# ECP-ExaGraph/miniVite

Hardware: NVIDIA B200
Metric: louvain_phase_edges_per_sec (higher is better)
Workload: dtype f64

## Files before the change

__graft_entry__.py:

```python
import os
import subprocess
import sys

ROOT = os.path.dirname(os.path.abspath(__file__))
PKG = os.path.join(ROOT, "minivite_b200")
CSRC = os.path.join(PKG, "csrc")
LIBDIR = os.path.join(PKG, "lib")
BINDIR = os.path.join(ROOT, "bin")
if ROOT not in sys.path:
    sys.path.insert(0, ROOT)

NVCC_FLAGS = ["-gencode", "arch=compute_100a,code=sm_100a", "-lineinfo", "-O3", "-std=c++17", "-fmad=false",
              "-Xcompiler", "-fPIC,-ffp-contract=off,-pthread"]
HOST_FLAGS = ["-std=c++17", "-O3", "-fopenmp", "-ffp-contract=off", "-fPIC", "-Wall"]


def _newer(target, sources):
    if not os.path.exists(target):
        return True
    t = os.path.getmtime(target)
    return any(os.path.getmtime(s) > t for s in sources)


def _srcs(*rel):
    return [os.path.join(CSRC, r) for r in rel]


def build_host_only():
    os.makedirs(LIBDIR, exist_ok=True)
    host_src = _srcs("host/hostlib.cpp", "host/rgg.hpp", "host/graph.hpp", "host/binio.hpp")
    out = os.path.join(LIBDIR, "libmvhost.so")
    if _newer(out, host_src):
        subprocess.check_call(["g++"] + HOST_FLAGS + ["-shared", "-o", out, host_src[0]])
    from oracle import oracle as O
    O.build()


def build():
    import fcntl
    os.makedirs(LIBDIR, exist_ok=True)
    lk = os.open(os.path.join(LIBDIR, ".build.lock"), os.O_RDONLY | os.O_CREAT, 0o644)
    try:
        fcntl.flock(lk, fcntl.LOCK_EX)
        _build_locked()
    finally:
        os.close(lk)


def _build_locked():
    build_host_only()
    inc = os.path.join(ROOT, "include", "mvgpu.h")
    cu_src = _srcs("mvgpu.cu", "narrow.cpp", "kernels.cuh", "scan_pipe.cuh", "rgg_gpu.cuh", "nccl_dyn.h") + [inc]
    out = os.path.join(LIBDIR, "libmvgpu.so")
    if _newer(out, cu_src):
        subprocess.check_call(["nvcc"] + NVCC_FLAGS + ["-shared", "-o", out, cu_src[0], cu_src[1], "-ldl", "-lpthread"])
    main_src = _srcs("host/main.cpp", "host/louvain.hpp", "host/rgg.hpp", "host/graph.hpp", "host/binio.hpp") + [inc]
    if all(os.path.exists(s) for s in main_src):
        os.makedirs(BINDIR, exist_ok=True)
        exe = os.path.join(BINDIR, "miniVite_b200")
        if _newer(exe, main_src + [out]):
            subprocess.check_call(["g++"] + HOST_FLAGS + ["-I", os.path.join(ROOT, "include"), "-o", exe, main_src[0],
                                                         "-L", LIBDIR, "-lmvgpu", "-Wl,-rpath,$ORIGIN/../minivite_b200/lib"])
    if os.path.isdir("/root/reference"):
        subprocess.check_call([sys.executable, os.path.join(ROOT, "oracle", "build_ref.py"), "--gpu"])
    import minivite_b200
    from minivite_b200 import gpu, hostgraph
    hostgraph.lib()
    L = gpu.lib()
    for name in gpu.EXPORTS:
        getattr(L, name)


def smoke():
    build()
    import numpy as np
    from minivite_b200 import gpu, hostgraph
    from oracle import oracle as O
    ss = hostgraph.generate_rgg(16384, 1)
    sh = ss.shards[0]
    g = gpu.LouvainGPU(0, 0, 1)
    g.set_option("trace", 1)
    g.upload(sh.nv, sh.parts, sh.rowptr, sh.edges)
    mod, iters = g.louvain(-1.0, 1.0e-6)
    comm = g.communities()
    tr = g.trace()
# ... 14 lines not shown
```

include/mvgpu.h:

```cpp
#ifndef MVGPU_H
#define MVGPU_H

#include <stdint.h>

#ifdef __cplusplus
extern "C" {
#endif

typedef struct mvgpu_ctx mvgpu_ctx;

#define MVGPU_UNIQUE_ID_BYTES 128

typedef struct {
  double modularity;
  int64_t moved;
  uint64_t chash;
} mvgpu_iter_trace;

typedef struct {
  double total_s;
  double setup_s;
  double scan_s;
  double fold_s;
  double exchange_s;
// ... 8 lines not shown
  int64_t h2d_bytes;
} mvgpu_timings;

const char *mvgpu_last_error(void);
int mvgpu_device_count(void);

int mvgpu_create(mvgpu_ctx **ctx, int device, int rank, int nranks);
int mvgpu_destroy(mvgpu_ctx *ctx);

int mvgpu_get_unique_id(void *id128);
int mvgpu_comm_init(mvgpu_ctx *ctx, const void *id128);

int mvgpu_upload_shard(mvgpu_ctx *ctx, int64_t nv_global, const int64_t *parts, int64_t lnv, int64_t lne,
                       const int64_t *edge_indices, const void *edge_list);
int mvgpu_attach_shard_device(mvgpu_ctx *ctx, int64_t nv_global, const int64_t *parts, int64_t lnv, int64_t lne,
                              const int64_t *d_edge_indices, const void *d_edge_list);

int mvgpu_generate_rgg_shard(mvgpu_ctx *ctx, int64_t nv_global, int unit_weight, int64_t *lne_out);
int mvgpu_generate_rgg_shard_ex(mvgpu_ctx *ctx, int64_t nv_global, int unit_weight, int lcg, double random_edge_percent,
                                int64_t *lne_out);
int mvgpu_download_shard(mvgpu_ctx *ctx, int64_t *edge_indices, void *edge_list);

int mvgpu_louvain(mvgpu_ctx *ctx, double lower, double thresh, int *iters, double *modularity);

int mvgpu_get_communities(mvgpu_ctx *ctx, int64_t *out);
int mvgpu_get_communities_device(mvgpu_ctx *ctx, const int32_t **d_out);

int mvgpu_set_option(mvgpu_ctx *ctx, const char *name, int64_t value);
int mvgpu_get_trace(mvgpu_ctx *ctx, int max_entries, mvgpu_iter_trace *out, int *n);
int mvgpu_get_timings(mvgpu_ctx *ctx, mvgpu_timings *out);
int mvgpu_get_scan_times(mvgpu_ctx *ctx, int max_entries, double *out, int *n);
int mvgpu_get_constant(mvgpu_ctx *ctx, double *out);
int mvgpu_get_shard_info(mvgpu_ctx *ctx, int64_t *info6);

int mvgpu_upload_shard32(mvgpu_ctx *ctx, int32_t nv_global, const int32_t *parts, int32_t lnv, int32_t lne,
                         const int32_t *edge_indices, const void *edge_list8);
int mvgpu_louvain32(mvgpu_ctx *ctx, float lower, float thresh, int *iters, float *modularity);
int mvgpu_get_communities32(mvgpu_ctx *ctx, int32_t *out);

int mvgpu_dist_louvain_method(int device, int64_t nv, int64_t ne_local, const int64_t *edge_indices,
                              const void *edge_list, double lower, double thresh, int *iters,
                              double *modularity, int64_t *comm_out);

#ifdef __cplusplus
}
#endif
#endif
```

minivite_b200/csrc/kernels.cuh:

```cuda
#pragma once
#include <cooperative_groups.h>
#include <cuda_runtime.h>
#include <stdint.h>

namespace mv {

#ifndef MV_TILE_V
#define MV_TILE_V 128
#endif
#ifndef MV_ECAP
#define MV_ECAP 2048
#endif
constexpr int kTileV = MV_TILE_V;
constexpr int kECap = MV_ECAP;
#ifndef MV_STAGE_U
#define MV_STAGE_U 6
#endif
constexpr int kStageU = MV_STAGE_U;
constexpr int kMaxRanks = 16;

struct Edge16 { long long tail; double weight; };
struct CommW { long long size; double degree; };

struct Acc {
// ... 748 lines not shown
    } else {
      double tw = 0.0, sl = 0.0;
      for (uint32_t e = e0; e < e1; e++) {
        const double w = weights[e];
        tw += w;
        if (tails[e] == v) sl += w;
      }
      vdeg[v] = tw;
      self_d[v] = (double)(long long)sl;
      any_self |= (sl != 0.0);
      CommW c; c.size = 1; c.degree = tw;
      cinfo_w[v] = c;
      usize[v] = 0; udeg[v] = 0.0;
      tw_sum += tw;
    }
  }
  tw_sum = warp_sum(tw_sum);
  if (UNIT) sq_sum = warp_sum(sq_sum);
  any_self = __any_sync(0xffffffffu, any_self);
  if (bad) *unordered = 1;
  if ((threadIdx.x & 31) == 0) {
    if (UNIT && sq_sum) atomicAdd(&acc0->la2_u, sq_sum);
    if (tw_sum != 0.0) atomicAdd(total_weight, tw_sum);
    if (any_self) atomicOr(has_self, 1u);
  }
}

__global__ void __launch_bounds__(256) k_collect_heavy(int lnv, const uint32_t *rowptr, unsigned int heavy_deg, int32_t *list,
                                                       unsigned int *count) {
  for (int v = blockIdx.x * blockDim.x + threadIdx.x; v < lnv; v += gridDim.x * blockDim.x)
    if (rowptr[v + 1] - rowptr[v] > heavy_deg) list[atomicAdd(count, 1u)] = v;
}

#ifndef MV_BFS_SUB
#define MV_BFS_SUB 4
#endif
constexpr unsigned int kBfsRegionBits = 22;
constexpr unsigned int kBfsUnreached = 0xFFFFFFFFu;

__global__ void __launch_bounds__(256) k_msbfs(int lnv, const uint32_t *rowptr, const int32_t *tails, uint32_t *key,
                                               int region_stride, int max_levels, unsigned int *level_flags) {
  namespace cg = cooperative_groups;
  cg::grid_group grid = cg::this_grid();
  const int gtid = blockIdx.x * blockDim.x + threadIdx.x, gsz = gridDim.x * blockDim.x;
  for (int v = gtid; v < lnv; v += gsz)
    key[v] = (v % region_stride == 0) ? (unsigned int)(v / region_stride) : kBfsUnreached;
  grid.sync();
  const int lane = threadIdx.x & 31;
  constexpr int kBfsSub = MV_BFS_SUB, kBfsLanes = 32 / kBfsSub;
  __shared__ uint32_t s_front[256 / 32][32][3];
  uint32_t(*front)[3] = s_front[threadIdx.x >> 5];
  for (int level = 0; level < max_levels; level++) {
    bool any = false;
    for (int vb = (gtid - lane); vb < lnv; vb += gsz) {
      const int v = vb + lane;
      unsigned int k = kBfsUnreached;
      if (v < lnv) k = __ldcg(key + v);
      const bool active = (k != kBfsUnreached) && ((k >> kBfsRegionBits) == (unsigned int)level);
      const unsigned int m = __ballot_sync(0xffffffffu, active);
      if (m == 0) continue;
      any = true;
      if (active) {
        const int slot = __popc(m & ((1u << lane) - 1u));
        front[slot][0] = ((unsigned int)(level + 1) << kBfsRegionBits) | (k & ((1u << kBfsRegionBits) - 1));
        front[slot][1] = rowptr[v];
        front[slot][2] = rowptr[v + 1];
      }
      __syncwarp();
      const int cnt = __popc(m);
      for (int i = lane / kBfsLanes; i < cnt; i += kBfsSub) {
        const unsigned int nk = front[i][0];
        const uint32_t e1 = front[i][2];
        for (uint32_t e = front[i][1] + (lane % kBfsLanes); e < e1; e += kBfsLanes) {
          const int w = tails[e];
          if (w < lnv && __ldcg(key + w) > nk) atomicMin(&key[w], nk);
        }
      }
      __syncwarp();
    }
    if (__syncthreads_or(any) && threadIdx.x == 0) level_flags[level] = 1;
    grid.sync();
    if (__ldcg(level_flags + level) == 0) break;
  }
}

constexpr unsigned int kBfsLevelBits = 8;
__global__ void __launch_bounds__(256) k_bfs_sortkeys(int lnv, const uint32_t *key, uint32_t *sortkey, int32_t *ids,
                                                      unsigned int unreached_key) {
  for (int v = blockIdx.x * blockDim.x + threadIdx.x; v < lnv; v += gridDim.x * blockDim.x) {
    const unsigned int k = key[v];
    unsigned int sk;
    if (k == kBfsUnreached) sk = unreached_key;
    else {
      const unsigned int region = k & ((1u << kBfsRegionBits) - 1), level = min(k >> kBfsRegionBits, (1u << kBfsLevelBits) - 1u);
      sk = (region << kBfsLevelBits) | level;
    }
    sortkey[v] = sk;
    ids[v] = v;
  }
}

__global__ void __launch_bounds__(256) k_perm_inverse(int lnv, const int32_t *perm, long long base, int32_t *inv, int32_t *lab,
                                                      const uint32_t *rowptr_old, uint32_t *deg_new) {
  for (int i = blockIdx.x * blockDim.x + threadIdx.x; i <= lnv; i += gridDim.x * blockDim.x) {
    if (i == lnv) { deg_new[i] = 0; continue; }
    const int o = perm[i];
    inv[o] = i;
    lab[i] = (int32_t)(base + o);
    deg_new[i] = rowptr_old[o + 1] - rowptr_old[o];
  }
}

__global__ void __launch_bounds__(256) k_permute_adj(int lnv, const int32_t *perm, const int32_t *inv, const uint32_t *rowptr_old,
                                                     const int32_t *tails_old, const double *w_old, const uint32_t *rowptr_new,
                                                     int32_t *tails_new, double *w_new, int nlow, unsigned int *unordered) {
  const int lane = threadIdx.x & 7;
  const int tile = (blockIdx.x * blockDim.x + threadIdx.x) >> 3, ntiles = (gridDim.x * blockDim.x) >> 3;
  bool bad = false;
  for (int i = tile; i < lnv; i += ntiles) {
    const int o = perm[i];
    const uint32_t s0 = rowptr_old[o], s1 = rowptr_old[o + 1], d0 = rowptr_new[i];
    for (uint32_t k = lane; k < s1 - s0; k += 8) {
      const int t = tails_old[s0 + k];
      if (k && !tails_ascend(tails_old[s0 + k - 1], t, lnv, nlow)) bad = true;
      tails_new[d0 + k] = (t < lnv) ? inv[t] : t;
      if (w_old) w_new[d0 + k] = w_old[s0 + k];
    }
  }
  if (bad) *unordered = 1;
}

__global__ void __launch_bounds__(256) k_span_sample(int lnv, const uint32_t *rowptr, const int32_t *tails, int stride,
                                                     unsigned long long *span_sum, unsigned long long *span_cnt) {
  unsigned long long s = 0, c = 0;
  for (int v = (blockIdx.x * blockDim.x + threadIdx.x) * stride; v < lnv; v += gridDim.x * blockDim.x * stride) {
    const uint32_t e1 = rowptr[v + 1];
    for (uint32_t e = rowptr[v]; e < e1; e++) {
      const int t = tails[e];
      if (t < lnv) { s += (unsigned long long)abs(t - v); c++; }
    }
  }
  s = warp_sum(s); c = warp_sum(c);
  if ((threadIdx.x & 31) == 0 && c) { atomicAdd(span_sum, s); atomicAdd(span_cnt, c); }
}

template <bool MULTI>
__global__ void __launch_bounds__(256) k_final_labels(int lnv, const int32_t *cur, const int32_t *perm, ScanParams p, int32_t *out) {
  for (int i = blockIdx.x * blockDim.x + threadIdx.x; i < lnv; i += gridDim.x * blockDim.x) {
    const int c = cur[i];
    out[perm ? perm[i] : i] = label_of<MULTI>(p, c);
  }
}

struct P2PState {
  unsigned long long arrive[kMaxRanks];
  unsigned long long vals[2][kMaxRanks][4];
  unsigned int error;
  unsigned int pad_;
};
// ... 89 lines not shown
```

minivite_b200/csrc/mvgpu.cu:

```cuda
#include <cuda_runtime.h>
#include <unistd.h>

#include <algorithm>
#include <atomic>
#include <cmath>
#include <cstdio>
#include <cstring>
#include <cub/cub.cuh>
#include <random>
#include <string>
#include <thread>
#include <vector>

#include "../../include/mvgpu.h"
#include "host_comm.hpp"
#include "kernels.cuh"
#include "scan_pipe.cuh"
#include "scan_queue.cuh"
#include "nccl_dyn.h"
#include "rgg_gpu.cuh"

extern "C" void mv_narrow_edges(const void *edge_records, long long n, long long nv, long long base, long long bound,
                                int32_t *dst, long long *nremote, int *bad);

// ... 58 lines not shown
  int device = 0, rank = 0, nranks = 1;
  cudaStream_t stream = nullptr;
  int num_sms = 148;
  ncclComm_t comm = nullptr;
  mvhost::HostComm hc;
  long long nv_global = 0, lnv = 0, lne = 0, base = 0, bound = 0;
  std::vector<long long> parts;
  const long long *d_rowptr64 = nullptr;
  const Edge16 *d_edges = nullptr;
  DevBuf<long long> in_rowptr;
  DevBuf<Edge16> in_edges;
  DevBuf<long long> gen_rowptr;
  DevBuf<Edge16> gen_edges;
  DevBuf<int32_t> in_tails32;
  DevBuf<Edge16> raw_ring;
  long long raw_chunks = 0;
  DevBuf<long long> wide;
  void *h_bounce[2] = {nullptr, nullptr};
  const int32_t *d_tails32 = nullptr;
  long long in_nremote = 0;
  void *h_stage = nullptr;
  size_t h_stage_cap = 0;
  const uint32_t *a_rowptr = nullptr;
  const int32_t *a_tails = nullptr;
  const double *a_weights = nullptr;
  bool have_graph = false;
  DevBuf<uint32_t> rowptr;
  DevBuf<int32_t> tails;
  DevBuf<double> weights;
  DevBuf<int32_t> self_i;
  DevBuf<uint32_t> bfs_key, sortkey, sortkey2, deg_new, rowptr2;
  DevBuf<int32_t> ids, perm, inv, lab, tails2, final_orig;
  DevBuf<double> weights2;
  DevBuf<unsigned int> level_flags;
  bool reordered = false;
  int relabel = 0;
  double reorder_s = 0.0;
  DevBuf<double> self_d, vdeg;
  DevBuf<int32_t> comm_a, comm_b;
  DevBuf<uint32_t> cdeg;
  DevBuf<int32_t> csize;
  DevBuf<unsigned long long> upd;
  DevBuf<CommW> cinfo_w;
  DevBuf<long long> usize;
  DevBuf<double> udeg;
  DevBuf<Acc> acc;
  DevBuf<unsigned char> scratch;
  DevBuf<unsigned char> cub_tmp, coll_tmp;
  DevBuf<long long> sorted_tmp;
  DevBuf<long long> remote_list, ghost_gid, send_gid;
  DevBuf<uint32_t> remote_pos;
  DevBuf<int32_t> send_lid, send_buf;
  long long nghost = 0, nsend = 0;
  std::vector<long long> rcount, scount, roff, soff;
  DevBuf<int32_t> heavy_list, hkeys, hvals_i;
  DevBuf<double> hvals_d;
  DevBuf<unsigned long long> heavy_off;
  long long nheavy = 0, maxdeg = 0;
  int scan_has_self = 0, scan_heavy_deg = kECap;
  int scan_kernel = 4;
  bool simple_sorted = false;
  DevBuf<P2PState> p2p;
  P2PPeers pp;
  PushTable push[2];
  unsigned long long p2p_epoch = 0;
  bool p2p_zeroed = false;
  int32_t *peer_comm[2][kMaxRanks];
// ... 410 lines not shown
    TRY(coll_alltoallv_dev(c, c->ghost_gid.p, c->rcount, c->roff, c->send_gid.p, c->scount, c->soff, sizeof(long long)));
    if (c->nsend) {
      k_gid_to_lid<<<grid_for(c->nsend, 256, nsm), 256, 0, s>>>(c->send_gid.p, (int)c->nsend, c->base, c->send_lid.p);
      c->tm.kernel_launches++;
    }
  }

  c->reordered = false;
  c->relabel = 0;
  {
    int want = c->opt_reorder == 1 ? 1 : 0;
    if (c->opt_reorder == 2 && lnv >= 65536) {
      k_span_sample<<<grid_for(lnv / 64 + 1, 256, nsm), 256, 0, s>>>((int)lnv, src_rowptr, src_tails, 64, &d_sc->span_sum, &d_sc->span_cnt);
      c->tm.kernel_launches++;
      unsigned long long sp2[2];
      CK(cudaMemcpyAsync(sp2, &d_sc->span_sum, sizeof sp2, cudaMemcpyDeviceToHost, s));
      CK(cudaStreamSynchronize(s));
      if (sp2[1] > 0 && (double)sp2[0] / (double)sp2[1] > (double)lnv / 64.0) want = 1;
    }
    int any = want;
    if (c->nranks > 1) {
      long long hv = want;
      TRY(coll_allreduce_i64(c, &hv, 1, true));
      any = hv != 0;
    }
    c->relabel = any;
    if (any && lnv > 0) {
      cudaEvent_t r0 = get_event(c, 2), r1 = get_event(c, 3);
      CK(cudaEventRecord(r0, s));
      TRY(c->perm.ensure(lnv)); TRY(c->inv.ensure(lnv)); TRY(c->lab.ensure(lnv)); TRY(c->ids.ensure(lnv));
      TRY(c->bfs_key.ensure(lnv)); TRY(c->sortkey.ensure(lnv)); TRY(c->sortkey2.ensure(lnv));
      TRY(c->deg_new.ensure(lnv + 1)); TRY(c->rowptr2.ensure(lnv + 1 + 40)); TRY(c->tails2.ensure(lne + 4));
      if (!c->unit) TRY(c->weights2.ensure(lne + 4));
      const int max_levels = 1023;
      TRY(c->level_flags.ensure(max_levels + 1));
      CK(cudaMemsetAsync(c->level_flags.p, 0, sizeof(unsigned int) * (max_levels + 1), s));
      if (want) {
        int occ = 0;
        CK(cudaOccupancyMaxActiveBlocksPerMultiprocessor(&occ, k_msbfs, 256, 0));
        if (occ < 1) return fail("k_msbfs cannot be made resident");
        int ilnv = (int)lnv, stride = c->opt_region, ml = max_levels;
        const uint32_t *rp = src_rowptr; const int32_t *tl = src_tails; uint32_t *key = c->bfs_key.p; unsigned int *lf = c->level_flags.p;
        void *args[] = {&ilnv, &rp, &tl, &key, &stride, &ml, &lf};
        CK(cudaLaunchCooperativeKernel((void *)k_msbfs, dim3(occ * nsm), dim3(256), args, 0, s));
        const long long nregions = (lnv + stride - 1) / stride;
        int sort_bits = (int)kBfsLevelBits;
        while ((1LL << (sort_bits - (int)kBfsLevelBits)) <= nregions && sort_bits < 32) sort_bits++;
        const unsigned int unreached_key = sort_bits >= 32 ? 0xFFFFFFFFu : ((1u << sort_bits) - 1u);
        k_bfs_sortkeys<<<grid_for(lnv, 256, nsm), 256, 0, s>>>((int)lnv, c->bfs_key.p, c->sortkey.p, c->ids.p, unreached_key);
        size_t tb = 0;
        cub::DeviceRadixSort::SortPairs(nullptr, tb, c->sortkey.p, c->sortkey2.p, c->ids.p, c->perm.p, (int)lnv, 0, sort_bits, s);
        TRY(c->cub_tmp.ensure(tb));
        tb = c->cub_tmp.cap;
        CK(cub::DeviceRadixSort::SortPairs(c->cub_tmp.p, tb, c->sortkey.p, c->sortkey2.p, c->ids.p, c->perm.p, (int)lnv, 0, sort_bits, s));
        c->tm.kernel_launches += 3;
      } else {
        k_bfs_sortkeys<<<grid_for(lnv, 256, nsm), 256, 0, s>>>((int)lnv, c->bfs_key.p, c->sortkey.p, c->perm.p, 0xFFFFFFFFu);
        c->tm.kernel_launches++;
      }
      k_perm_inverse<<<grid_for(lnv + 1, 256, nsm), 256, 0, s>>>((int)lnv, c->perm.p, c->base, c->inv.p, c->lab.p, src_rowptr, c->deg_new.p);
      c->tm.kernel_launches++;
      if (want) {
        size_t tb = 0;
        cub::DeviceScan::ExclusiveSum(nullptr, tb, c->deg_new.p, c->rowptr2.p, (int)lnv + 1, s);
        TRY(c->cub_tmp.ensure(tb));
        tb = c->cub_tmp.cap;
        CK(cub::DeviceScan::ExclusiveSum(c->cub_tmp.p, tb, c->deg_new.p, c->rowptr2.p, (int)lnv + 1, s));
        k_permute_adj<<<grid_for(lnv * 8, 256, nsm, 16), 256, 0, s>>>((int)lnv, c->perm.p, c->inv.p, src_rowptr, src_tails, src_weights,
                                                                    c->rowptr2.p, c->tails2.p, c->unit ? nullptr : c->weights2.p,
                                                                    (int)c->roff[c->rank], &d_sc->unordered);
        c->tm.kernel_launches += 2;
        src_rowptr = c->rowptr2.p;
        src_tails = c->tails2.p;
        src_weights = c->unit ? nullptr : c->weights2.p;
        c->reordered = true;
      }
      CK(cudaEventRecord(r1, s));
    }
    if (c->relabel && c->nsend) {
      k_apply_inv<<<grid_for(c->nsend, 256, nsm), 256, 0, s>>>(c->send_lid.p, (int)c->nsend, c->inv.p);
      c->tm.kernel_launches++;
    }
  }

  c->a_rowptr = src_rowptr; c->a_tails = src_tails; c->a_weights = src_weights;

  const long long nslots = lnv + c->nghost;
  TRY(c->comm_a.ensure(std::max(nslots, lnv + nremote)));
  TRY(c->comm_b.ensure(std::max(nslots, lnv + nremote)));
  if (c->unit) { TRY(c->cdeg.ensure(lnv)); TRY(c->csize.ensure(lnv)); TRY(c->upd.ensure(lnv)); TRY(c->self_i.ensure(lnv)); }
  else { TRY(c->cinfo_w.ensure(lnv)); TRY(c->usize.ensure(lnv)); TRY(c->udeg.ensure(lnv)); TRY(c->vdeg.ensure(lnv)); TRY(c->self_d.ensure(lnv)); }
  TRY(c->acc.ensure((size_t)c->opt_max_iters + 2));
  CK(cudaMemsetAsync(c->acc.p, 0, sizeof(Acc) * ((size_t)c->opt_max_iters + 2), s));

  if (c->unit)
    k_vertex_init<true><<<grid_for(lnv, 256, nsm), 256, 0, s>>>((int)lnv, c->base, c->a_rowptr, c->a_tails, nullptr, c->comm_a.p,
                                                              c->cdeg.p, c->csize.p, c->upd.p, nullptr, nullptr, nullptr, nullptr,
                                                              c->self_i.p, nullptr, &d_sc->total_weight, &d_sc->has_self,
                                                              (int)c->roff[c->rank], c->reordered ? nullptr : &d_sc->unordered, c->acc.p);
  else
    k_vertex_init<false><<<grid_for(lnv, 256, nsm), 256, 0, s>>>((int)lnv, c->base, c->a_rowptr, c->a_tails, c->a_weights, c->comm_a.p,
// ... 357 lines not shown
      const std::string kv = all.substr(pos, end - pos);
      pos = end + 1;
      const size_t eq = kv.find('=');
      if (kv.empty()) continue;
      if (eq == std::string::npos || mvgpu_set_option(c, kv.substr(0, eq).c_str(), atoll(kv.c_str() + eq + 1))) {
        const std::string msg = "MVGPU_OPTIONS: bad entry '" + kv + "'" + (eq == std::string::npos ? "" : ": " + g_err);
        mvgpu_destroy(c);
        return fail(msg);
      }
    }
  }
  *out = c;
  return 0;
}

int mvgpu_destroy(mvgpu_ctx *c) {
  if (!c) return 0;
  cudaSetDevice(c->device);
  if (c->stream) cudaStreamSynchronize(c->stream);
  for (void *p : c->ipc_opened) cudaIpcCloseMemHandle(p);
  if (c->comm) g_nccl.CommDestroy(c->comm);
  c->hc.close_comm();
  for (cudaEvent_t e : c->events) cudaEventDestroy(e);
  if (c->h_stage) cudaFreeHost(c->h_stage);
  c->in_tails32.release(); c->wide.release(); c->raw_ring.release();
  for (int b = 0; b < 2; b++) if (c->h_bounce[b]) cudaFreeHost(c->h_bounce[b]);
  c->gen_rowptr.release(); c->gen_edges.release();
  c->in_rowptr.release(); c->in_edges.release(); c->rowptr.release(); c->tails.release(); c->weights.release();
  c->self_i.release(); c->self_d.release(); c->vdeg.release(); c->comm_a.release(); c->comm_b.release();
  c->cdeg.release(); c->csize.release(); c->upd.release(); c->cinfo_w.release(); c->usize.release(); c->udeg.release(); c->acc.release();
  c->scratch.release(); c->cub_tmp.release(); c->coll_tmp.release(); c->sorted_tmp.release(); c->remote_list.release(); c->remote_pos.release(); c->ghost_gid.release(); c->send_gid.release();
  c->bfs_key.release(); c->sortkey.release(); c->sortkey2.release(); c->deg_new.release(); c->rowptr2.release();
  c->ids.release(); c->perm.release(); c->inv.release(); c->lab.release(); c->tails2.release(); c->final_orig.release();
  c->weights2.release(); c->level_flags.release();
  c->p2p.release();
  c->send_lid.release(); c->send_buf.release(); c->heavy_list.release(); c->hkeys.release(); c->hvals_i.release();
  c->hvals_d.release(); c->heavy_off.release();
  if (c->h_pin) cudaFreeHost(c->h_pin);
  if (c->stream) cudaStreamDestroy(c->stream);
  delete c;
  return 0;
}

int mvgpu_get_unique_id(void *id128) {
  static_assert(sizeof(ncclUniqueId) == MVGPU_UNIQUE_ID_BYTES, "ncclUniqueId size");
  if (!mvnccl::load(g_nccl, g_err)) {
    FILE *f = fopen("/dev/urandom", "rb");
    if (!f || fread(id128, 1, MVGPU_UNIQUE_ID_BYTES, f) != MVGPU_UNIQUE_ID_BYTES) { if (f) fclose(f); return 1; }
    fclose(f);
    return 0;
  }
  ncclUniqueId id;
  NK(g_nccl.GetUniqueId(&id));
  memcpy(id128, &id, sizeof id);
  return 0;
}

int mvgpu_comm_init(mvgpu_ctx *c, const void *id128) {
  if (!c) return fail("null ctx");
  if (c->nranks == 1) return 0;
  if (c->opt_host_transport) {
    std::string err;
    if (c->hc.open(id128, c->rank, c->nranks, err)) return fail(err);
    return 0;
  }
  if (!mvnccl::load(g_nccl, g_err)) return 1;
  CK(cudaSetDevice(c->device));
// ... 360 lines not shown
  if (!c || !n) return fail("null argument");
  const int k = std::min<int>(max_entries, (int)c->trace.size());
  if (out && k > 0) memcpy(out, c->trace.data(), sizeof(mvgpu_iter_trace) * k);
  *n = (int)c->trace.size();
  return 0;
}

int mvgpu_get_scan_times(mvgpu_ctx *c, int max_entries, double *out, int *n) {
  if (!c || !n) return fail("null argument");
  const int k = std::min<int>(max_entries, (int)c->scan_times.size());
  if (out && k > 0) memcpy(out, c->scan_times.data(), sizeof(double) * k);
  *n = (int)c->scan_times.size();
  return 0;
}

int mvgpu_get_timings(mvgpu_ctx *c, mvgpu_timings *out) {
  if (!c || !out) return fail("null argument");
  *out = c->tm;
  return 0;
}

int mvgpu_get_constant(mvgpu_ctx *c, double *out) {
  if (!c || !out) return fail("null argument");
  *out = c->constant;
  return 0;
}

int mvgpu_get_shard_info(mvgpu_ctx *c, int64_t *info6) {
  if (!c || !info6) return fail("null argument");
  info6[0] = c->lnv; info6[1] = c->lne; info6[2] = c->nghost; info6[3] = c->nsend; info6[4] = c->nheavy; info6[5] = c->maxdeg;
  return 0;
}

int mvgpu_upload_shard32(mvgpu_ctx *c, int32_t nv_global, const int32_t *parts, int32_t lnv, int32_t lne,
                         const int32_t *edge_indices, const void *edge_list8) {
  if (!c || !parts || !edge_indices || (lne && !edge_list8)) return fail("null argument");
  CK(cudaSetDevice(c->device));
  std::vector<int64_t> parts64(parts, parts + c->nranks + 1);
  TRY(set_graph(c, nv_global, parts64.data(), lnv, lne));
  c->f32 = true;
  DevBuf<Edge8> e8;
  DevBuf<int32_t> rp32;
  TRY(e8.ensure((size_t)lne)); TRY(rp32.ensure((size_t)lnv + 1));
  TRY(c->in_edges.ensure(lne)); TRY(c->in_rowptr.ensure(lnv + 1));
  cudaEvent_t a = get_event(c, 0), b = get_event(c, 1);
  CK(cudaEventRecord(a, c->stream));
  CK(cudaMemcpyAsync(rp32.p, edge_indices, sizeof(int32_t) * ((size_t)lnv + 1), cudaMemcpyHostToDevice, c->stream));
  if (lne) CK(cudaMemcpyAsync(e8.p, edge_list8, sizeof(Edge8) * (size_t)lne, cudaMemcpyHostToDevice, c->stream));
  k_widen_shard32<<<grid_for(std::max<long long>(lne, lnv + 1), 256, c->num_sms, 16), 256, 0, c->stream>>>(e8.p, lne, rp32.p, lnv, c->in_edges.p,
                                                                                                      c->in_rowptr.p);
  CK(cudaEventRecord(b, c->stream));
  CK(cudaEventSynchronize(b));
  float ms = 0;
  CK(cudaEventElapsedTime(&ms, a, b));
  c->h2d_s = ms * 1e-3;
  c->h2d_bytes = (long long)sizeof(int32_t) * (lnv + 1) + (long long)sizeof(Edge8) * lne;
  c->d_rowptr64 = c->in_rowptr.p;
  c->d_edges = c->in_edges.p;
  c->d_tails32 = nullptr;
  return 0;
}

int mvgpu_louvain32(mvgpu_ctx *c, float lower, float thresh, int *iters, float *modularity) {
  if (!c || !iters || !modularity) return fail("null argument");
  if (!c->f32) return fail("mvgpu_louvain32 needs a shard uploaded with mvgpu_upload_shard32");
  double mod = 0.0;
// ... 30 lines not shown
```

minivite_b200/gpu.py:

```python
import ctypes
import os

import numpy as np

_LIB_PATH = os.environ.get("MVGPU_LIB") or os.path.join(os.path.dirname(os.path.abspath(__file__)), "lib", "libmvgpu.so")
UNIQUE_ID_BYTES = 128

TRACE_DTYPE = np.dtype([("modularity", "<f8"), ("moved", "<i8"), ("chash", "<u8")])


class Timings(ctypes.Structure):
    _fields_ = [("total_s", ctypes.c_double), ("setup_s", ctypes.c_double), ("scan_s", ctypes.c_double),
                ("fold_s", ctypes.c_double), ("exchange_s", ctypes.c_double), ("h2d_s", ctypes.c_double),
                ("scan_launches", ctypes.c_int64), ("kernel_launches", ctypes.c_int64),
                ("iters", ctypes.c_int32), ("unit_weight", ctypes.c_int32), ("reorder_s", ctypes.c_double),
                ("reordered", ctypes.c_int32), ("scan_kernel_chosen", ctypes.c_int32), ("h2d_bytes", ctypes.c_int64)]

    def as_dict(self):
        return {k: getattr(self, k) for k, _ in self._fields_}


EXPORTS = ["mvgpu_last_error", "mvgpu_device_count", "mvgpu_create", "mvgpu_destroy", "mvgpu_get_unique_id",
           "mvgpu_comm_init", "mvgpu_upload_shard", "mvgpu_attach_shard_device", "mvgpu_generate_rgg_shard", "mvgpu_generate_rgg_shard_ex",
           "mvgpu_download_shard", "mvgpu_louvain",
           "mvgpu_get_communities", "mvgpu_get_communities_device", "mvgpu_upload_shard32", "mvgpu_louvain32", "mvgpu_get_communities32", "mvgpu_set_option", "mvgpu_get_trace",
           "mvgpu_get_timings", "mvgpu_get_scan_times", "mvgpu_get_constant", "mvgpu_get_shard_info", "mvgpu_dist_louvain_method"]

_lib = None


def lib():
    global _lib
    if _lib is None:
        if not os.path.exists(_LIB_PATH):
            raise RuntimeError(f"{_LIB_PATH} missing: the CUDA extension is not built "
                               "(python -c 'import __graft_entry__ as g; g.build()'); there is no CPU fallback")
        L = ctypes.CDLL(_LIB_PATH)
        vp, i64, dbl, ci = ctypes.c_void_p, ctypes.c_int64, ctypes.c_double, ctypes.c_int
        L.mvgpu_last_error.restype = ctypes.c_char_p
        L.mvgpu_create.argtypes = [ctypes.POINTER(vp), ci, ci, ci]
        L.mvgpu_destroy.argtypes = [vp]
        L.mvgpu_get_unique_id.argtypes = [vp]
        L.mvgpu_comm_init.argtypes = [vp, vp]
        L.mvgpu_upload_shard.argtypes = [vp, i64, vp, i64, i64, vp, vp]
        L.mvgpu_attach_shard_device.argtypes = [vp, i64, vp, i64, i64, vp, vp]
        L.mvgpu_generate_rgg_shard.argtypes = [vp, i64, ci, ctypes.POINTER(i64)]
        L.mvgpu_generate_rgg_shard_ex.argtypes = [vp, i64, ci, ci, ctypes.c_double, ctypes.POINTER(i64)]
        L.mvgpu_download_shard.argtypes = [vp, vp, vp]
        L.mvgpu_louvain.argtypes = [vp, dbl, dbl, ctypes.POINTER(ci), ctypes.POINTER(dbl)]
        L.mvgpu_get_communities.argtypes = [vp, vp]
        L.mvgpu_upload_shard32.argtypes = [vp, ctypes.c_int32, vp, ctypes.c_int32, ctypes.c_int32, vp, vp]
        L.mvgpu_louvain32.argtypes = [vp, ctypes.c_float, ctypes.c_float, ctypes.POINTER(ci), ctypes.POINTER(ctypes.c_float)]
        L.mvgpu_get_communities32.argtypes = [vp, vp]
        L.mvgpu_get_communities_device.argtypes = [vp, ctypes.POINTER(vp)]
        L.mvgpu_set_option.argtypes = [vp, ctypes.c_char_p, i64]
        L.mvgpu_get_trace.argtypes = [vp, ci, vp, ctypes.POINTER(ci)]
        L.mvgpu_get_timings.argtypes = [vp, ctypes.POINTER(Timings)]
        L.mvgpu_get_scan_times.argtypes = [vp, ci, vp, ctypes.POINTER(ci)]
        L.mvgpu_get_constant.argtypes = [vp, ctypes.POINTER(dbl)]
        L.mvgpu_get_shard_info.argtypes = [vp, vp]
        L.mvgpu_dist_louvain_method.argtypes = [ci, i64, i64, vp, vp, dbl, dbl, ctypes.POINTER(ci),
                                                ctypes.POINTER(dbl), vp]
        _lib = L
    return _lib


class MvgpuError(RuntimeError):
    pass


def _ck(rc):
    if rc != 0:
        raise MvgpuError(lib().mvgpu_last_error().decode(errors="replace"))


def device_count():
    n = lib().mvgpu_device_count()
    if n < 0:
        raise MvgpuError(lib().mvgpu_last_error().decode(errors="replace"))
    return n


def get_unique_id():
    buf = ctypes.create_string_buffer(UNIQUE_ID_BYTES)
    _ck(lib().mvgpu_get_unique_id(buf))
    return buf.raw


class LouvainGPU:

    def __init__(self, device=0, rank=0, nranks=1):
        self._h = ctypes.c_void_p()
        self.rank, self.nranks, self.device = rank, nranks, device
# ... 76 lines not shown
        _ck(lib().mvgpu_get_communities(self._h, out.ctypes.data))
        return out[:self.lnv]

    def trace(self):
        n = ctypes.c_int(0)
        _ck(lib().mvgpu_get_trace(self._h, 0, None, ctypes.byref(n)))
        out = np.zeros(n.value, dtype=TRACE_DTYPE)
        if n.value:
            _ck(lib().mvgpu_get_trace(self._h, n.value, out.ctypes.data, ctypes.byref(n)))
        return out

    def timings(self):
        t = Timings()
        _ck(lib().mvgpu_get_timings(self._h, ctypes.byref(t)))
        return t.as_dict()

    def scan_times(self):
        n = ctypes.c_int(0)
        _ck(lib().mvgpu_get_scan_times(self._h, 0, None, ctypes.byref(n)))
        out = np.zeros(n.value, dtype=np.float64)
        if n.value:
            _ck(lib().mvgpu_get_scan_times(self._h, n.value, out.ctypes.data, ctypes.byref(n)))
        return out

    def constant(self):
        v = ctypes.c_double(0)
        _ck(lib().mvgpu_get_constant(self._h, ctypes.byref(v)))
        return v.value

    def shard_info(self):
        info = (ctypes.c_int64 * 6)()
        _ck(lib().mvgpu_get_shard_info(self._h, info))
        return dict(zip(["lnv", "lne", "nghost", "nsend", "nheavy", "maxdeg"], [int(x) for x in info]))

    def close(self):
        if self._h:
            lib().mvgpu_destroy(self._h)
            self._h = ctypes.c_void_p()

    def __del__(self):
        try:
            self.close()
        except Exception:
            pass


def dist_louvain_method(me, nprocs, shard, lower=-1.0, thresh=1.0e-6, device=None, unique_id=None, want_comm=False):
    g = LouvainGPU(device if device is not None else me, me, nprocs)
    try:
        if nprocs > 1:
            g.comm_init(unique_id)
        g.upload(shard.nv, shard.parts, shard.rowptr, shard.edges)
        mod, iters = g.louvain(lower, thresh)
        if want_comm:
            return mod, iters, g.communities()
        return mod, iters
    finally:
        g.close()
```

Measured before the change: 191.9 billion.

## Replace level-scan multi-source BFS with frontier-queue BFS and warp-balanced adjacency permute

The reordering BFS used to rescan every vertex at every level to find the active frontier. It now keeps explicit frontier queues, with warp-level load-balanced edge expansion and claims staged in shared memory. Once the frontier becomes small, the remaining levels finish in a single CTA, so small levels avoid grid-wide syncs. The adjacency permutation kernel is rewritten so each warp handles 32 rows with load-balanced edge distribution instead of eight lanes per row. A permutation-export API is also added. Claiming vertices via atomicMin can change which region wins compared with the previous relaxation, and that could alter the ordering.

```diff
diff --git a/__graft_entry__.py b/__graft_entry__.py
--- a/__graft_entry__.py
+++ b/__graft_entry__.py
@@ -50,7 +50,8 @@
 def _build_locked():
     build_host_only()
     inc = os.path.join(ROOT, "include", "mvgpu.h")
-    cu_src = _srcs("mvgpu.cu", "narrow.cpp", "kernels.cuh", "scan_pipe.cuh", "rgg_gpu.cuh", "nccl_dyn.h") + [inc]
+    cu_src = _srcs("mvgpu.cu", "narrow.cpp", "kernels.cuh", "scan_pipe.cuh", "scan_queue.cuh", "rgg_gpu.cuh", "nccl_dyn.h",
+                    "host_comm.hpp") + [inc]
     out = os.path.join(LIBDIR, "libmvgpu.so")
     if _newer(out, cu_src):
         subprocess.check_call(["nvcc"] + NVCC_FLAGS + ["-shared", "-o", out, cu_src[0], cu_src[1], "-ldl", "-lpthread"])
diff --git a/include/mvgpu.h b/include/mvgpu.h
--- a/include/mvgpu.h
+++ b/include/mvgpu.h
@@ -64,6 +64,7 @@
 int mvgpu_get_scan_times(mvgpu_ctx *ctx, int max_entries, double *out, int *n);
 int mvgpu_get_constant(mvgpu_ctx *ctx, double *out);
 int mvgpu_get_shard_info(mvgpu_ctx *ctx, int64_t *info6);
+int mvgpu_get_permutation(mvgpu_ctx *ctx, int32_t *perm_out);
 
 int mvgpu_upload_shard32(mvgpu_ctx *ctx, int32_t nv_global, const int32_t *parts, int32_t lnv, int32_t lne,
                          const int32_t *edge_indices, const void *edge_list8);
diff --git a/minivite_b200/csrc/kernels.cuh b/minivite_b200/csrc/kernels.cuh
--- a/minivite_b200/csrc/kernels.cuh
+++ b/minivite_b200/csrc/kernels.cuh
@@ -804,55 +804,117 @@
     if (rowptr[v + 1] - rowptr[v] > heavy_deg) list[atomicAdd(count, 1u)] = v;
 }
 
-#ifndef MV_BFS_SUB
-#define MV_BFS_SUB 4
-#endif
 constexpr unsigned int kBfsRegionBits = 22;
 constexpr unsigned int kBfsUnreached = 0xFFFFFFFFu;
-
-__global__ void __launch_bounds__(256) k_msbfs(int lnv, const uint32_t *rowptr, const int32_t *tails, uint32_t *key,
-                                               int region_stride, int max_levels, unsigned int *level_flags) {
+#ifndef MV_BFS_TAIL_CTA
+#define MV_BFS_TAIL_CTA 1024
+#endif
+constexpr int kBfsUnroll = 4;
+
+__device__ __forceinline__ int owner_lane(unsigned int off, unsigned int j) {
+  int q = 0;
+#pragma unroll
+  for (int step = 16; step; step >>= 1)
+    if (__shfl_sync(0xffffffffu, off, q + step) <= j) q += step;
+  return q;
+}
+
+constexpr unsigned int kBfsStage = 256;
+__device__ __forceinline__ void bfs_flush(int32_t *stage, unsigned int staged, int32_t *next, unsigned int *next_count) {
+  const int lane = threadIdx.x & 31;
+  __syncwarp();
+  unsigned int base = 0;
+  if (lane == 0) base = atomicAdd(next_count, staged);
+  base = __shfl_sync(0xffffffffu, base, 0);
+  for (unsigned int i = lane; i < staged; i += 32) next[base + i] = stage[i];
+  __syncwarp();
+}
+
+__device__ __forceinline__ void bfs_expand(int lnv, const uint32_t *rowptr, const int32_t *tails, uint32_t *key, int level,
+                                           const int32_t *cur, unsigned int n, int32_t *next, unsigned int *next_count,
+                                           int warp, int nwarps, int32_t *stage) {
+  const int lane = threadIdx.x & 31;
+  const unsigned int lanes_below = (1u << lane) - 1u;
+  unsigned int staged = 0;
+  for (unsigned int b = (unsigned int)warp * 32; b < n; b += (unsigned int)nwarps * 32) {
+    unsigned int nk = 0, s0 = 0, len = 0;
+    if (b + lane < n) {
+      const int v = __ldcg(cur + b + lane);
+      nk = ((unsigned int)(level + 1) << kBfsRegionBits) | (__ldcg(key + v) & ((1u << kBfsRegionBits) - 1));
+      s0 = rowptr[v];
+      len = rowptr[v + 1] - s0;
+    }
+    unsigned int off = len;
+#pragma unroll
+    for (int d = 1; d < 32; d <<= 1) {
+      const unsigned int x = __shfl_up_sync(0xffffffffu, off, d);
+      if (lane >= d) off += x;
+    }
+    const unsigned int total = __shfl_sync(0xffffffffu, off, 31);
+    off -= len;
+    for (unsigned int j0 = 0; j0 < total; j0 += 32 * kBfsUnroll) {
+      int w[kBfsUnroll];
+      unsigned int k[kBfsUnroll], probe[kBfsUnroll];
+#pragma unroll
+      for (int u = 0; u < kBfsUnroll; u++) {
+        const unsigned int j = j0 + u * 32 + lane;
+        const int q = owner_lane(off, j);
+        const unsigned int e = __shfl_sync(0xffffffffu, s0, q) + j - __shfl_sync(0xffffffffu, off, q);
+        k[u] = __shfl_sync(0xffffffffu, nk, q);
+        w[u] = j < total ? tails[e] : lnv;
+      }
+#pragma unroll
+      for (int u = 0; u < kBfsUnroll; u++) probe[u] = w[u] < lnv ? __ldcg(key + w[u]) : 0u;
+      unsigned int pos[kBfsUnroll], claimed = 0;
+#pragma unroll
+      for (int u = 0; u < kBfsUnroll; u++) {
+        const bool claim = probe[u] > k[u] && atomicMin(key + w[u], k[u]) == kBfsUnreached;
+        const unsigned int m = __ballot_sync(0xffffffffu, claim);
+        pos[u] = claim ? claimed + __popc(m & lanes_below) : 0xFFFFFFFFu;
+        claimed += __popc(m);
+      }
+      if (staged + claimed > kBfsStage) {
+        bfs_flush(stage, staged, next, next_count);
+        staged = 0;
+      }
+#pragma unroll
+      for (int u = 0; u < kBfsUnroll; u++)
+        if (pos[u] != 0xFFFFFFFFu) stage[staged + pos[u]] = w[u];
+      staged += claimed;
+    }
+  }
+  if (staged) bfs_flush(stage, staged, next, next_count);
+}
+
+__global__ void __launch_bounds__(256) k_bfs(int lnv, const uint32_t *rowptr, const int32_t *tails, uint32_t *key,
+                                             int region_stride, int max_levels, int32_t *qa, int32_t *qb,
+                                             unsigned int *count) {
   namespace cg = cooperative_groups;
   cg::grid_group grid = cg::this_grid();
+  __shared__ int32_t s_stage[256 / 32][kBfsStage];
+  int32_t *stage = s_stage[threadIdx.x >> 5];
   const int gtid = blockIdx.x * blockDim.x + threadIdx.x, gsz = gridDim.x * blockDim.x;
+  const unsigned int nseeds = (unsigned int)((lnv - 1) / region_stride + 1);
   for (int v = gtid; v < lnv; v += gsz)
     key[v] = (v % region_stride == 0) ? (unsigned int)(v / region_stride) : kBfsUnreached;
+  for (unsigned int i = gtid; i < nseeds; i += gsz) qa[i] = (int)(i * region_stride);
+  if (gtid == 0) count[0] = nseeds;
   grid.sync();
-  const int lane = threadIdx.x & 31;
-  constexpr int kBfsSub = MV_BFS_SUB, kBfsLanes = 32 / kBfsSub;
-  __shared__ uint32_t s_front[256 / 32][32][3];
-  uint32_t(*front)[3] = s_front[threadIdx.x >> 5];
-  for (int level = 0; level < max_levels; level++) {
-    bool any = false;
-    for (int vb = (gtid - lane); vb < lnv; vb += gsz) {
-      const int v = vb + lane;
-      unsigned int k = kBfsUnreached;
-      if (v < lnv) k = __ldcg(key + v);
-      const bool active = (k != kBfsUnreached) && ((k >> kBfsRegionBits) == (unsigned int)level);
-      const unsigned int m = __ballot_sync(0xffffffffu, active);
-      if (m == 0) continue;
-      any = true;
-      if (active) {
-        const int slot = __popc(m & ((1u << lane) - 1u));
-        front[slot][0] = ((unsigned int)(level + 1) << kBfsRegionBits) | (k & ((1u << kBfsRegionBits) - 1));
-        front[slot][1] = rowptr[v];
-        front[slot][2] = rowptr[v + 1];
-      }
-      __syncwarp();
-      const int cnt = __popc(m);
-      for (int i = lane / kBfsLanes; i < cnt; i += kBfsSub) {
-        const unsigned int nk = front[i][0];
-        const uint32_t e1 = front[i][2];
-        for (uint32_t e = front[i][1] + (lane % kBfsLanes); e < e1; e += kBfsLanes) {
-          const int w = tails[e];
-          if (w < lnv && __ldcg(key + w) > nk) atomicMin(&key[w], nk);
-        }
-      }
-      __syncwarp();
-    }
-    if (__syncthreads_or(any) && threadIdx.x == 0) level_flags[level] = 1;
+  int level = 0;
+  unsigned int n = nseeds, prev = 0xFFFFFFFFu;
+  for (; level < max_levels && n > 0 && !(n < MV_BFS_TAIL_CTA && n < prev && level > 0); level++) {
+    bfs_expand(lnv, rowptr, tails, key, level, (level & 1) ? qb : qa, n, (level & 1) ? qa : qb, count + level + 1, gtid >> 5, gsz >> 5,
+               stage);
     grid.sync();
-    if (__ldcg(level_flags + level) == 0) break;
+    prev = n;
+    n = __ldcg(count + level + 1);
+  }
+  if (blockIdx.x != 0) return;
+  for (; level < max_levels && n > 0; level++) {
+    bfs_expand(lnv, rowptr, tails, key, level, (level & 1) ? qb : qa, n, (level & 1) ? qa : qb, count + level + 1,
+               threadIdx.x >> 5, blockDim.x >> 5, stage);
+    __syncthreads();
+    n = __ldcg(count + level + 1);
   }
 }
 
@@ -883,20 +945,49 @@
   }
 }
 
+constexpr int kPermUnroll = 4;
 __global__ void __launch_bounds__(256) k_permute_adj(int lnv, const int32_t *perm, const int32_t *inv, const uint32_t *rowptr_old,
                                                      const int32_t *tails_old, const double *w_old, const uint32_t *rowptr_new,
                                                      int32_t *tails_new, double *w_new, int nlow, unsigned int *unordered) {
-  const int lane = threadIdx.x & 7;
-  const int tile = (blockIdx.x * blockDim.x + threadIdx.x) >> 3, ntiles = (gridDim.x * blockDim.x) >> 3;
+  const int lane = threadIdx.x & 31;
+  const int warp = (blockIdx.x * blockDim.x + threadIdx.x) >> 5, nwarps = (gridDim.x * blockDim.x) >> 5;
   bool bad = false;
-  for (int i = tile; i < lnv; i += ntiles) {
-    const int o = perm[i];
-    const uint32_t s0 = rowptr_old[o], s1 = rowptr_old[o + 1], d0 = rowptr_new[i];
-    for (uint32_t k = lane; k < s1 - s0; k += 8) {
-      const int t = tails_old[s0 + k];
-      if (k && !tails_ascend(tails_old[s0 + k - 1], t, lnv, nlow)) bad = true;
-      tails_new[d0 + k] = (t < lnv) ? inv[t] : t;
-      if (w_old) w_new[d0 + k] = w_old[s0 + k];
+  for (int i0 = warp * 32; i0 < lnv; i0 += nwarps * 32) {
+    const uint32_t d0 = rowptr_new[i0], total = rowptr_new[min(i0 + 32, lnv)] - d0;
+    uint32_t s0 = 0, off = total;
+    if (i0 + lane < lnv) {
+      s0 = rowptr_old[perm[i0 + lane]];
+      off = rowptr_new[i0 + lane] - d0;
+    }
+    for (uint32_t j0 = 0; j0 < total; j0 += 32 * kPermUnroll) {
+      uint32_t e[kPermUnroll];
+      bool first[kPermUnroll];
+      int t[kPermUnroll], prev[kPermUnroll], r[kPermUnroll];
+#pragma unroll
+      for (int u = 0; u < kPermUnroll; u++) {
+        const uint32_t j = j0 + u * 32 + lane;
+        const int q = owner_lane(off, j);
+        const uint32_t oq = __shfl_sync(0xffffffffu, off, q);
+        e[u] = __shfl_sync(0xffffffffu, s0, q) + j - oq;
+        first[u] = j == oq;
+      }
+#pragma unroll
+      for (int u = 0; u < kPermUnroll; u++) {
+        const bool valid = j0 + u * 32 + lane < total;
+        t[u] = valid ? tails_old[e[u]] : 0;
+        prev[u] = valid && !first[u] ? tails_old[e[u] - 1] : -1;
+      }
+#pragma unroll
+      for (int u = 0; u < kPermUnroll; u++) r[u] = (t[u] < lnv) ? inv[t[u]] : t[u];
+#pragma unroll
+      for (int u = 0; u < kPermUnroll; u++) {
+        const uint32_t j = j0 + u * 32 + lane;
+        if (j < total) {
+          if (prev[u] >= 0 && !tails_ascend(prev[u], t[u], lnv, nlow)) bad = true;
+          tails_new[d0 + j] = r[u];
+          if (w_old) w_new[d0 + j] = w_old[e[u]];
+        }
+      }
     }
   }
   if (bad) *unordered = 1;
diff --git a/minivite_b200/csrc/mvgpu.cu b/minivite_b200/csrc/mvgpu.cu
--- a/minivite_b200/csrc/mvgpu.cu
+++ b/minivite_b200/csrc/mvgpu.cu
@@ -114,7 +114,7 @@
   DevBuf<uint32_t> bfs_key, sortkey, sortkey2, deg_new, rowptr2;
   DevBuf<int32_t> ids, perm, inv, lab, tails2, final_orig;
   DevBuf<double> weights2;
-  DevBuf<unsigned int> level_flags;
+  DevBuf<unsigned int> bfs_count;
   bool reordered = false;
   int relabel = 0;
   double reorder_s = 0.0;
@@ -591,17 +591,18 @@
       TRY(c->bfs_key.ensure(lnv)); TRY(c->sortkey.ensure(lnv)); TRY(c->sortkey2.ensure(lnv));
       TRY(c->deg_new.ensure(lnv + 1)); TRY(c->rowptr2.ensure(lnv + 1 + 40)); TRY(c->tails2.ensure(lne + 4));
       if (!c->unit) TRY(c->weights2.ensure(lne + 4));
-      const int max_levels = 1023;
-      TRY(c->level_flags.ensure(max_levels + 1));
-      CK(cudaMemsetAsync(c->level_flags.p, 0, sizeof(unsigned int) * (max_levels + 1), s));
       if (want) {
+        const int max_levels = 1023;
+        TRY(c->bfs_count.ensure(max_levels + 1));
+        CK(cudaMemsetAsync(c->bfs_count.p, 0, sizeof(unsigned int) * (max_levels + 1), s));
         int occ = 0;
-        CK(cudaOccupancyMaxActiveBlocksPerMultiprocessor(&occ, k_msbfs, 256, 0));
-        if (occ < 1) return fail("k_msbfs cannot be made resident");
+        CK(cudaOccupancyMaxActiveBlocksPerMultiprocessor(&occ, k_bfs, 256, 0));
+        if (occ < 1) return fail("k_bfs cannot be made resident");
         int ilnv = (int)lnv, stride = c->opt_region, ml = max_levels;
-        const uint32_t *rp = src_rowptr; const int32_t *tl = src_tails; uint32_t *key = c->bfs_key.p; unsigned int *lf = c->level_flags.p;
-        void *args[] = {&ilnv, &rp, &tl, &key, &stride, &ml, &lf};
-        CK(cudaLaunchCooperativeKernel((void *)k_msbfs, dim3(occ * nsm), dim3(256), args, 0, s));
+        const uint32_t *rp = src_rowptr; const int32_t *tl = src_tails; uint32_t *key = c->bfs_key.p;
+        int32_t *qa = c->ids.p, *qb = c->perm.p; unsigned int *cnt = c->bfs_count.p;
+        void *args[] = {&ilnv, &rp, &tl, &key, &stride, &ml, &qa, &qb, &cnt};
+        CK(cudaLaunchCooperativeKernel((void *)k_bfs, dim3(occ * nsm), dim3(256), args, 0, s));
         const long long nregions = (lnv + stride - 1) / stride;
         int sort_bits = (int)kBfsLevelBits;
         while ((1LL << (sort_bits - (int)kBfsLevelBits)) <= nregions && sort_bits < 32) sort_bits++;
@@ -625,7 +626,7 @@
         TRY(c->cub_tmp.ensure(tb));
         tb = c->cub_tmp.cap;
         CK(cub::DeviceScan::ExclusiveSum(c->cub_tmp.p, tb, c->deg_new.p, c->rowptr2.p, (int)lnv + 1, s));
-        k_permute_adj<<<grid_for(lnv * 8, 256, nsm, 16), 256, 0, s>>>((int)lnv, c->perm.p, c->inv.p, src_rowptr, src_tails, src_weights,
+        k_permute_adj<<<grid_for(lnv, 256, nsm, 16), 256, 0, s>>>((int)lnv, c->perm.p, c->inv.p, src_rowptr, src_tails, src_weights,
                                                                     c->rowptr2.p, c->tails2.p, c->unit ? nullptr : c->weights2.p,
                                                                     (int)c->roff[c->rank], &d_sc->unordered);
         c->tm.kernel_launches += 2;
@@ -1049,7 +1050,7 @@
   c->scratch.release(); c->cub_tmp.release(); c->coll_tmp.release(); c->sorted_tmp.release(); c->remote_list.release(); c->remote_pos.release(); c->ghost_gid.release(); c->send_gid.release();
   c->bfs_key.release(); c->sortkey.release(); c->sortkey2.release(); c->deg_new.release(); c->rowptr2.release();
   c->ids.release(); c->perm.release(); c->inv.release(); c->lab.release(); c->tails2.release(); c->final_orig.release();
-  c->weights2.release(); c->level_flags.release();
+  c->weights2.release(); c->bfs_count.release();
   c->p2p.release();
   c->send_lid.release(); c->send_buf.release(); c->heavy_list.release(); c->hkeys.release(); c->hvals_i.release();
   c->hvals_d.release(); c->heavy_off.release();
@@ -1476,6 +1477,14 @@
   return 0;
 }
 
+int mvgpu_get_permutation(mvgpu_ctx *c, int32_t *perm_out) {
+  if (!c || !perm_out) return fail("null argument");
+  if (!c->d_final || !c->reordered) return fail("the last run did not renumber its vertices");
+  CK(cudaMemcpyAsync(perm_out, c->perm.p, sizeof(int32_t) * c->lnv, cudaMemcpyDeviceToHost, c->stream));
+  CK(cudaStreamSynchronize(c->stream));
+  return 0;
+}
+
 int mvgpu_upload_shard32(mvgpu_ctx *c, int32_t nv_global, const int32_t *parts, int32_t lnv, int32_t lne,
                          const int32_t *edge_indices, const void *edge_list8) {
   if (!c || !parts || !edge_indices || (lne && !edge_list8)) return fail("null argument");
diff --git a/minivite_b200/gpu.py b/minivite_b200/gpu.py
--- a/minivite_b200/gpu.py
+++ b/minivite_b200/gpu.py
@@ -24,7 +24,7 @@
            "mvgpu_comm_init", "mvgpu_upload_shard", "mvgpu_attach_shard_device", "mvgpu_generate_rgg_shard", "mvgpu_generate_rgg_shard_ex",
            "mvgpu_download_shard", "mvgpu_louvain",
            "mvgpu_get_communities", "mvgpu_get_communities_device", "mvgpu_upload_shard32", "mvgpu_louvain32", "mvgpu_get_communities32", "mvgpu_set_option", "mvgpu_get_trace",
-           "mvgpu_get_timings", "mvgpu_get_scan_times", "mvgpu_get_constant", "mvgpu_get_shard_info", "mvgpu_dist_louvain_method"]
+           "mvgpu_get_timings", "mvgpu_get_scan_times", "mvgpu_get_constant", "mvgpu_get_shard_info", "mvgpu_get_permutation", "mvgpu_dist_louvain_method"]
 
 _lib = None
 
@@ -59,6 +59,7 @@
         L.mvgpu_get_scan_times.argtypes = [vp, ci, vp, ctypes.POINTER(ci)]
         L.mvgpu_get_constant.argtypes = [vp, ctypes.POINTER(dbl)]
         L.mvgpu_get_shard_info.argtypes = [vp, vp]
+        L.mvgpu_get_permutation.argtypes = [vp, vp]
         L.mvgpu_dist_louvain_method.argtypes = [ci, i64, i64, vp, vp, dbl, dbl, ctypes.POINTER(ci),
                                                 ctypes.POINTER(dbl), vp]
         _lib = L
@@ -201,6 +202,11 @@
         info = (ctypes.c_int64 * 6)()
         _ck(lib().mvgpu_get_shard_info(self._h, info))
         return dict(zip(["lnv", "lne", "nghost", "nsend", "nheavy", "maxdeg"], [int(x) for x in info]))
+
+    def permutation(self):
+        out = np.empty(self.lnv, dtype=np.int32)
+        _ck(lib().mvgpu_get_permutation(self._h, out.ctypes.data))
+        return out
 
     def close(self):
         if self._h:
```

New measurement: 204.5 billion (median of 6 runs). 1.07x the previous value.
